# noirmist/Pytorch_Pose_Proposal_Network

Measured on AMD Instinct MI355X. Metric: images/sec (384x384, DRN-D-22) at 1/2/4/8 MI355X, higher is better.
Workload: dtype bf16

## Files before the change

pytorch_pose_proposal_network_amd/csrc/conv_big.hip:

```cpp
#include <algorithm>
#include <cstdio>
#include <cstdlib>
#include <type_traits>
#include <utility>

#include "conv_common.h"

namespace {

using namespace ppnconv;

constexpr bool stats_tile_ok(int bp, int bc) {
    return bc >= 128 && (size_t)bp * (size_t)(bc * 2 + 16) <= 2 * (size_t)(bp + bc) * 128;
}

#ifndef PPN_DIAG
#define PPN_DIAG 0
#endif
constexpr unsigned kOOB = 0x80000000u;

template <typename F, int... I>
__device__ __forceinline__ void static_for_impl(F&& f, std::integer_sequence<int, I...>) {
    (f(std::integral_constant<int, I>{}), ...);
}
template <int N, typename F>
__device__ __forceinline__ void static_for(F&& f) {
    static_for_impl(f, std::make_integer_sequence<int, N>{});
}

template <typename T>
__device__ __forceinline__ void load4(const char* p, float* v);
template <>
__device__ __forceinline__ void load4<float>(const char* p, float* v) {
    const float4 a = *reinterpret_cast<const float4*>(p);
    v[0] = a.x; v[1] = a.y; v[2] = a.z; v[3] = a.w;
}
template <>
__device__ __forceinline__ void load4<__bf16>(const char* p, float* v) {
    const uint2 a = *reinterpret_cast<const uint2*>(p);
    v[0] = __uint_as_float(a.x << 16); v[1] = __uint_as_float(a.x & 0xffff0000u);
    v[2] = __uint_as_float(a.y << 16); v[3] = __uint_as_float(a.y & 0xffff0000u);
}
template <>
__device__ __forceinline__ void load4<_Float16>(const char* p, float* v) {
    typedef __attribute__((ext_vector_type(4))) _Float16 f16x4;
    const f16x4 a = *reinterpret_cast<const f16x4*>(p);
#pragma unroll
    for (int i = 0; i < 4; ++i) v[i] = (float)a[i];
}
template <typename T>
__device__ __forceinline__ void store4(char* p, const float* v);
template <>
__device__ __forceinline__ void store4<float>(char* p, const float* v) {
    *reinterpret_cast<float4*>(p) = make_float4(v[0], v[1], v[2], v[3]);
}
template <>
__device__ __forceinline__ void store4<__bf16>(char* p, const float* v) {
    typedef __attribute__((ext_vector_type(4))) __bf16 bf16x4;
    bf16x4 o;
#pragma unroll
    for (int i = 0; i < 4; ++i) o[i] = (__bf16)v[i];
    *reinterpret_cast<bf16x4*>(p) = o;
}

template <>
__device__ __forceinline__ void store4<_Float16>(char* p, const float* v) {
    typedef __attribute__((ext_vector_type(4))) _Float16 f16x4;
    f16x4 o;
#pragma unroll
    for (int i = 0; i < 4; ++i) o[i] = (_Float16)clamp_f16(v[i]);
    *reinterpret_cast<f16x4*>(p) = o;
}

__device__ __forceinline__ void bufload_lds16(__amdgpu_buffer_rsrc_t rsrc, char* lds_wave_base, unsigned voff,
                                              unsigned soff) {
    __builtin_amdgcn_raw_ptr_buffer_load_lds(rsrc, (void __attribute__((address_space(3)))*)lds_wave_base, 16, voff,
                                             soff, 0, 0);
}

template <typename T, int BP, int BC, int NW, bool SC, bool X3 = false, bool ST = false, bool SP = false>
__global__ void __launch_bounds__(64 * NW, (ST && BP == 192 && BC == 128) ? 4 : NW / 4)
conv_igemm_big_kernel(ConvKArgs a, unsigned src_bytes, unsigned wgt_bytes) {
    static_assert(!X3 || (std::is_same<T, _Float16>::value && !SC), "X3 is the split-f16 mode without a fused shortcut");
    static_assert(!ST || (sizeof(T) == 2 && !SC && !X3 && NW == 8 && BC >= 128), "ST: plain 16-bit launches of the 8-wave tiles");
    static_assert(!SP || (sizeof(T) == 2 && BP == 192 && BC == 256 && NW == 8 && !SC && !X3 && !ST), "SP: the plain 16-bit 192 x 256 tile");
    constexpr int EPC = Elem<T>::EPC;
    constexpr int BK = 8 * EPC;
    constexpr int ES = sizeof(T);
    constexpr int NT = 64 * NW;
    constexpr int WC = (BP % (16 * (NW / 2)) == 0) ? 2 : NW;
    constexpr int WP = NW / WC;
    constexpr int NXI = (BP + 8 * NW - 1) / (8 * NW), NWI = BC / (8 * NW);
    constexpr bool XRAGGED = BP % (8 * NW) != 0;
    constexpr int TP = BP / WP / 16, TC = BC / WC / 16;
    constexpr int STAGE = (BP + BC) * 128;
    static_assert(BP % 8 == 0 && BC % (8 * NW) == 0 && (BP / WP) % 16 == 0 && BC % (16 * WC) == 0, "tile shape");
    static_assert(TP <= 9 && TC <= 8 && TC * TP % 2 == 0, "accumulators must fit the register file");

    extern __shared__ __attribute__((aligned(16))) char smem[];
#ifdef PPN_CLOCK
    const unsigned long long ck_entry = __builtin_amdgcn_s_memtime();
    const unsigned long long rk_entry = __builtin_amdgcn_s_memrealtime();
#endif
    const int tid = threadIdx.x, lane = tid & 63;
    const int wave = __builtin_amdgcn_readfirstlane(tid >> 6);
    const int wc = wave / WP, wp = wave % WP;

    int ptile, ctile;
    {
        const int nb = gridDim.x, id = blockIdx.x;
        const int xcd = id & 7, loc = id >> 3, q = nb >> 3, r = nb & 7;
        const int logical = (xcd < r ? xcd * (q + 1) : r * (q + 1) + (xcd - r) * q) + loc;
        ptile = fast_div(logical, a.div_nct);
        ctile = logical - ptile * a.n_ctiles;
    }
    const int m0 = a.m_base + ptile * BP, c0 = ctile * BC;

    const __amdgpu_buffer_rsrc_t xrs = __builtin_amdgcn_make_buffer_rsrc((void*)a.src, 0, src_bytes, 0x00020000);
    const __amdgpu_buffer_rsrc_t wrs = __builtin_amdgcn_make_buffer_rsrc((void*)a.wgt, 0, wgt_bytes, 0x00020000);
    const __amdgpu_buffer_rsrc_t xrs2 =
        __builtin_amdgcn_make_buffer_rsrc((void*)(SC ? a.src2 : a.src), 0, SC ? a.src2_bytes : 0u, 0x00020000);

    const int lrow = lane >> 3;
    const int chunk = (lane & 7) ^ (((lane >> 4) & 3) | ((wave & 1) << 2));
    const int ntaps = a.ks * a.ks;
    int xbase[NXI];
    int xbase2[NXI];
    unsigned xmask[NXI];
#pragma unroll
    for (int j = 0; j < NXI; ++j) {
        const int row = (j * NW + wave) * 8 + lrow;
        const int m = m0 + row;
        const bool vm = m < a.M;
        const int mm = vm ? m : 0;
        const int b = fast_div(mm, a.div_howo), rem = mm - b * a.HoWo;
        const int oy = fast_div(rem, a.div_wo), ox = rem - oy * a.Wo;
        const int iy0 = oy * a.stride - a.pad, ix0 = ox * a.stride - a.pad;
        xbase[j] = (((b * a.H + iy0) * a.W + ix0) * a.Cin + chunk * EPC) * ES;
        unsigned mk = 0, cx = 0;
#pragma unroll
        for (int dx = 0; dx < 5; ++dx)
            cx |= (dx < a.ks && (unsigned)(ix0 + dx * a.dil) < (unsigned)a.W) ? (1u << dx) : 0u;
#pragma unroll
        for (int dy = 0; dy < 5; ++dy)
            mk |= (dy < a.ks && (unsigned)(iy0 + dy * a.dil) < (unsigned)a.H) ? (cx << (dy * a.ks)) : 0u;
        mk = vm ? mk : 0u;
        xmask[j] = mk | (vm ? 0x80000000u : 0u);
        if constexpr (SC)
            xbase2[j] = (((b * a.H2 + oy * a.stride2) * a.W2 + ox * a.stride2) * a.Cin2 + chunk * EPC) * ES;
        else
            xbase2[j] = 0;
    }
    unsigned woff[NWI];
#pragma unroll
    for (int j = 0; j < NWI; ++j) {
        const int row = (j * NW + wave) * 8 + lrow;
        woff[j] = (unsigned)(((size_t)(c0 + row) * a.Ktot + chunk * EPC) * ES);
    }

    constexpr int SBUF = 256 * 128;
    constexpr int NSP = 4;
    int sbase[NSP];
    unsigned smask = 0;
    int xoff[TP][3];
    if constexpr (SP) {
        const int P = a.sp_pitch;
        const int schunk = (lane & 7) ^ (lrow & 6);
        const int b0 = fast_div(m0, a.div_howo), oy0 = fast_div(m0 - b0 * a.HoWo, a.div_wo);
#pragma unroll
        for (int p = 0; p < NSP; ++p) {
            const int sr = (p * NW + wave) * 8 + lrow;
            const int r = fast_div(sr, a.sp_div), col = sr - r * P;
            const int iy0 = oy0 + r - a.dil, ix = col - a.dil;
            sbase[p] = (((b0 * a.H + iy0) * a.W + ix) * a.Cin + schunk * EPC) * ES;
            const bool colok = r < a.sp_rows && (unsigned)ix < (unsigned)a.W;
#pragma unroll
            for (int dy = 0; dy < 3; ++dy)
                smask |= (colok && (unsigned)(iy0 + dy * a.dil) < (unsigned)a.H) ? (1u << (3 * p + dy)) : 0u;
        }
        const int fr = lane & 15, fqq = lane >> 4;
#pragma unroll
        for (int j = 0; j < TP; ++j) {
            const int ml = wp * (BP / WP) + j * 16 + fr;
            const int r = fast_div(ml, a.div_wo), rb = r * P + (ml - r * a.Wo);
#pragma unroll
            for (int dx = 0; dx < 3; ++dx) {
                const int row = rb + dx * a.dil;
                xoff[j][dx] = row * 128 + ((fqq ^ (row & 6)) << 4);
            }
        }
    }

    const int nsteps = a.Ktot / BK;
    const int dx_bytes = a.dil * a.Cin * ES;
    const int dy_bytes = a.dil * a.W * a.Cin * ES - a.ks * dx_bytes;
    const int ksz = a.ks;
    int u_tap = 0, u_dx = 0, u_slab = 0, tapoff = 0, u_ph = 0;
    unsigned tapbit = 1u;
    unsigned ksoff = 0;
    bool live = true;
    bool phase2 = a.nsteps_main == 0;
    int ld_step = 0;
    auto advance = [&]() {
        ++ld_step;
        live = ld_step < nsteps;
        ksoff = live ? ksoff + BK * ES : 0u;
        const bool now2 = SC && ld_step >= a.nsteps_main;
        if (!now2) {
            ++u_tap; ++u_dx;
            tapoff += dx_bytes;
            const bool wrapx = u_dx == ksz;
            u_dx = wrapx ? 0 : u_dx;
            tapoff += wrapx ? dy_bytes : 0;
            const bool wrapt = u_tap == ntaps;
            u_tap = wrapt ? 0 : u_tap;
            if constexpr (X3) {
                u_ph += wrapt ? 1 : 0;
                const bool wrapp = u_ph == 3;
                u_ph = wrapp ? 0 : u_ph;
                u_slab += wrapp ? BK * ES : 0;
                tapoff = wrapt ? u_slab + (u_ph == 2 ? a.lo_off : 0) : tapoff;
            } else {
                u_slab += wrapt ? BK * ES : 0;
                tapoff = wrapt ? u_slab : tapoff;
            }
            tapbit = live ? (1u << u_tap) : 0u;
        } else {
            tapoff = phase2 ? tapoff + BK * ES : 0;
            tapbit = live ? 0x80000000u : 0u;
        }
        phase2 = now2;
    };
    auto issue_one = [&](auto gc, int buf) {
        constexpr int g = decltype(gc)::value;
        char* xs = smem + buf * STAGE;
        if constexpr (g < NXI) {
            if constexpr (XRAGGED && g == NXI - 1)
                if ((g * NW + wave) * 8 >= BP) return;
            if (!SC || !phase2) {
                const unsigned voff = (xmask[g] & tapbit) ? (unsigned)(xbase[g] + tapoff) : kOOB;
                bufload_lds16(xrs, xs + (g * NW + wave) * 1024, voff, 0);
            } else {
                const unsigned voff = (xmask[g] & tapbit) ? (unsigned)(xbase2[g] + tapoff) : kOOB;
                bufload_lds16(xrs2, xs + (g * NW + wave) * 1024, voff, 0);
            }
        } else {
            constexpr int j = g - NXI;
            bufload_lds16(wrs, xs + BP * 128 + (j * NW + wave) * 1024, live ? woff[j] : kOOB, ksoff);
        }
    };
    constexpr int NL = NXI + NWI;
    const int sp_dy_bytes = a.dil * a.W * a.Cin * ES;
    const int sp_nq = nsteps / 3;
    int sp_row = 0, sp_dy = 0, sp_slab = 0, sp_off = 0;
    unsigned sp_bit = 1u;
    auto sp_advance_row = [&]() {
        ++sp_row; ++sp_dy;
        sp_off += sp_dy_bytes;
        const bool wrap = sp_dy == 3;
        sp_dy = wrap ? 0 : sp_dy;
        sp_slab += wrap ? BK * ES : 0;
        sp_off = wrap ? sp_slab : sp_off;
        sp_bit = sp_row < sp_nq ? (1u << sp_dy) : 0u;
    };
    auto sp_advance_w = [&]() {
        ++ld_step;
        live = ld_step < nsteps;
        ksoff = live ? ksoff + BK * ES : 0u;
    };
    auto sp_issue_strip = [&](auto pc, int sb) {
        constexpr int p = decltype(pc)::value;
        const unsigned voff = ((smask >> (3 * p)) & sp_bit) ? (unsigned)(sbase[p] + sp_off) : kOOB;
        bufload_lds16(xrs, smem + sb + (p * NW + wave) * 1024, voff, 0);
    };
    auto sp_issue_w = [&](auto jc, int buf) {
        constexpr int j = decltype(jc)::value;
        bufload_lds16(wrs, smem + 2 * SBUF + buf * (BC * 128) + (j * NW + wave) * 1024, live ? woff[j] : kOOB, ksoff);
    };

    const int frow = lane & 15, fq = lane >> 4;
    const int fswz = (frow >> 1) & 7;
    int foff[2];
    foff[0] = frow * 128 + (((0 + fq) ^ fswz) << 4);
    foff[1] = frow * 128 + (((4 + fq) ^ fswz) << 4);
    const int x_tile_off = wp * (BP / WP) * 128;
    const int w_tile_off = BP * 128 + wc * (BC / WC) * 128;

    f32x4 acc[TC][TP];
#pragma unroll
    for (int i = 0; i < TC; ++i)
#pragma unroll
        for (int j = 0; j < TP; ++j) acc[i][j] = f32x4{0.f, 0.f, 0.f, 0.f};

    f32x4 wA[TC], xA[TP], wB[TC], xB[TP];
    constexpr int NRD = TC + TP;
    auto read_one = [&](auto rc, f32x4 (&wf)[TC], f32x4 (&xf)[TP], int buf, int ks) {
        constexpr int r = decltype(rc)::value;
#if PPN_DIAG == 6
        if (buf >= 0 && ks >= 0 && nsteps > 0) { asm volatile("" : "+v"(xf[0]), "+v"(wf[0])); return; }
#endif
        if constexpr (r < TP)
            xf[r] = *reinterpret_cast<const f32x4*>(smem + buf * STAGE + x_tile_off + foff[ks] + r * 16 * 128);
        else
            wf[r - TP] = *reinterpret_cast<const f32x4*>(smem + buf * STAGE + w_tile_off + foff[ks] + (r - TP) * 16 * 128);
    };
    auto sp_read_one = [&](auto rc, auto dxc, f32x4 (&wf)[TC], f32x4 (&xf)[TP], int wbuf, int xsel, int ks) {
        constexpr int r = decltype(rc)::value;
        constexpr int DX = decltype(dxc)::value;
        if constexpr (r < TP)
            xf[r] = *reinterpret_cast<const f32x4*>(smem + (xoff[r][DX] ^ xsel));
        else
            wf[r - TP] = *reinterpret_cast<const f32x4*>(smem + 2 * SBUF + wbuf * (BC * 128) + wc * (BC / WC) * 128 + foff[ks] +
                                                         (r - TP) * 16 * 128);
    };
    constexpr int GS = (TC * TP % 4 == 0) ? 4 : ((TC * TP % 3 == 0) ? 3 : 2);
    constexpr int NG = TC * TP / GS;
#if PPN_DIAG == 3 || PPN_DIAG == 4
    typedef float f32x16 __attribute__((ext_vector_type(16)));
    f32x16 acc32[TC * TP / 4];
#pragma unroll
    for (int i = 0; i < TC * TP / 4; ++i)
#pragma unroll
        for (int j = 0; j < 16; ++j) acc32[i][j] = 0.f;
#endif
    auto mma_group = [&](auto gc, const f32x4 (&wf)[TC], const f32x4 (&xf)[TP]) {
        constexpr int g = decltype(gc)::value;
#if PPN_DIAG == 3 || PPN_DIAG == 4
        if constexpr (std::is_same<T, __bf16>::value) {
            constexpr int i0 = g * 4, i1 = g * 4 + 3;
            acc32[g] = __builtin_amdgcn_mfma_f32_32x32x16_bf16(__builtin_bit_cast(bf16x8, wf[i0 / TP]),
                                                               __builtin_bit_cast(bf16x8, xf[i0 % TP]), acc32[g], 0, 0, 0);
            acc32[g] = __builtin_amdgcn_mfma_f32_32x32x16_bf16(__builtin_bit_cast(bf16x8, wf[i1 / TP]),
                                                               __builtin_bit_cast(bf16x8, xf[i1 % TP]), acc32[g], 0, 0, 0);
            return;
        }
#endif
        static_for<GS>([&](auto tc) {
            constexpr int idx = g * GS + decltype(tc)::value;
            mma_step(acc[idx / TP][idx % TP], wf[idx / TP], xf[idx % TP], (T*)nullptr);
        });
    };
    constexpr int RPG = (NRD + NG - 1) / NG;
    constexpr int LPG = (NL + NG - 1) / NG;

#ifdef PPN_CLOCK
    const unsigned long long ck_state = __builtin_amdgcn_s_memtime();
#endif
    if constexpr (SP) {
        static_for<NSP>([&](auto pc) { sp_issue_strip(pc, 0); });
        static_for<NWI>([&](auto jc) { sp_issue_w(jc, 0); });
        sp_advance_row();
        sp_advance_w();
        static_for<2>([&](auto pc) { sp_issue_strip(pc, SBUF); });
        static_for<NWI>([&](auto jc) { sp_issue_w(jc, 1); });
        sp_advance_w();
        asm volatile("s_waitcnt vmcnt(%0)" ::"n"(NWI + 2) : "memory");
    } else {
        static_for<NL>([&](auto gc) { issue_one(gc, 0); });
        advance();
        static_for<NL>([&](auto gc) { issue_one(gc, 1); });
        advance();
        if constexpr (XRAGGED) {
            if ((NXI - 1) * NW * 8 + wave * 8 < BP) asm volatile("s_waitcnt vmcnt(%0)" ::"n"(NL) : "memory");
            else asm volatile("s_waitcnt vmcnt(%0)" ::"n"(NL - 1) : "memory");
        } else {
            asm volatile("s_waitcnt vmcnt(%0)" ::"n"(NL) : "memory");
        }
    }
    __syncthreads();
#ifdef PPN_CLOCK
    const unsigned long long ck_bar = __builtin_amdgcn_s_memtime();
#endif
    if constexpr (SP) {
        constexpr std::integral_constant<int, 0> dx0{};
        static_for<NRD>([&](auto rc) { sp_read_one(rc, dx0, wA, xA, 0, 0, 0); });
        static_for<NRD>([&](auto rc) { sp_read_one(rc, dx0, wB, xB, 0, 64, 1); });
    } else {
        static_for<NRD>([&](auto rc) { read_one(rc, wA, xA, 0, 0); });
        static_for<NRD>([&](auto rc) { read_one(rc, wB, xB, 0, 1); });
    }
    static_for<NG>([&](auto gc) { mma_group(gc, wA, xA); });
    asm volatile("s_waitcnt vmcnt(0) lgkmcnt(0)" ::: "memory");
    __syncthreads();

#ifdef PPN_STAMP
    unsigned long long st_b1 = 0, st_b2 = 0, st_wait = 0, st_bar = 0, tq0, tq1;
#define PPN_T(var) do { __builtin_amdgcn_sched_barrier(0); asm volatile("s_memtime %0\n\ts_waitcnt lgkmcnt(0)" : "=s"(var) :: "memory"); __builtin_amdgcn_sched_barrier(0); } while (0)
#else
#define PPN_T(var) do { } while (0)
#endif
#ifdef PPN_CLOCK
    const unsigned long long ck0 = __builtin_amdgcn_s_memtime(), rk0 = __builtin_amdgcn_s_memrealtime();
#endif
    if constexpr (SP) {
        int s = 1, sbo = 0;
        auto step = [&](auto dxc) {
            constexpr int DX = decltype(dxc)::value;
            constexpr int NS = DX == 0 ? 2 : 1;
            const int buf = s & 1;
            static_for<NG>([&](auto gc) {
                constexpr int g = decltype(gc)::value;
                mma_group(gc, wB, xB);
                if constexpr (g < NS) sp_issue_strip(std::integral_constant<int, (DX == 0 ? g : DX + 1)>{}, sbo ^ SBUF);
                else if constexpr (g < NS + NWI) sp_issue_w(std::integral_constant<int, g - NS>{}, buf ^ 1);
                static_for<RPG>([&](auto rc) {
                    constexpr int r = g * RPG + decltype(rc)::value;
                    if constexpr (r < NRD) sp_read_one(std::integral_constant<int, r>{}, dxc, wA, xA, buf, sbo, 0);
                });
                __builtin_amdgcn_sched_barrier(0);
            });
            sp_advance_w();
            static_for<NG>([&](auto gc) {
                constexpr int g = decltype(gc)::value;
                mma_group(gc, wA, xA);
                static_for<RPG>([&](auto rc) {
                    constexpr int r = g * RPG + decltype(rc)::value;
                    if constexpr (r < NRD) sp_read_one(std::integral_constant<int, r>{}, dxc, wB, xB, buf, sbo | 64, 1);
                });
                __builtin_amdgcn_sched_barrier(0);
            });
            asm volatile("s_waitcnt vmcnt(0) lgkmcnt(0)" ::: "memory");
            __syncthreads();
            ++s;
        };
        static_assert(NG >= 2 + NWI, "one DMA per MFMA group");
        for (int q = 1; q < sp_nq; ++q) {
            step(std::integral_constant<int, 1>{});
            step(std::integral_constant<int, 2>{});
            sbo ^= SBUF;
            sp_advance_row();
            step(std::integral_constant<int, 0>{});
        }
        step(std::integral_constant<int, 1>{});
        step(std::integral_constant<int, 2>{});
    } else
    for (int s = 1; s < nsteps; ++s) {
        const int buf = s & 1;
#ifdef PPN_STAMP
        PPN_T(tq0);
#endif
        static_for<NG>([&](auto gc) {
            constexpr int g = decltype(gc)::value;
            mma_group(gc, wB, xB);
#if PPN_DIAG != 2 && PPN_DIAG != 4 && PPN_DIAG != 5 && PPN_DIAG != 6
            static_for<LPG>([&](auto lc) {
                constexpr int l = g * LPG + decltype(lc)::value;
                if constexpr (l < NL) issue_one(std::integral_constant<int, l>{}, buf ^ 1);
            });
#endif
            static_for<RPG>([&](auto rc) {
                constexpr int r = g * RPG + decltype(rc)::value;
                if constexpr (r < NRD) read_one(std::integral_constant<int, r>{}, wA, xA, buf, 0);
            });
            __builtin_amdgcn_sched_barrier(0);
        });
        advance();
#ifdef PPN_STAMP
        PPN_T(tq1); st_b1 += tq1 - tq0;
#endif
        static_for<NG>([&](auto gc) {
            constexpr int g = decltype(gc)::value;
            mma_group(gc, wA, xA);
            static_for<RPG>([&](auto rc) {
                constexpr int r = g * RPG + decltype(rc)::value;
                if constexpr (r < NRD) read_one(std::integral_constant<int, r>{}, wB, xB, buf, 1);
            });
            __builtin_amdgcn_sched_barrier(0);
        });
#ifdef PPN_STAMP
        PPN_T(tq0); st_b2 += tq0 - tq1;
#endif
#if PPN_DIAG == 1
        asm volatile("s_waitcnt lgkmcnt(0)" ::: "memory");
#else
        asm volatile("s_waitcnt vmcnt(0) lgkmcnt(0)" ::: "memory");
#endif
#ifdef PPN_STAMP
        PPN_T(tq1); st_wait += tq1 - tq0;
#endif
#if PPN_DIAG != 5
        __syncthreads();
#endif
#ifdef PPN_STAMP
        PPN_T(tq0); st_bar += tq0 - tq1;
#endif
    }
#ifdef PPN_CLOCK
    {
        const unsigned long long ck1 = __builtin_amdgcn_s_memtime(), rk1 = __builtin_amdgcn_s_memrealtime();
        if (lane == 0 && a.scale2 == nullptr && a.shift2 != nullptr) {
            unsigned long long* dbg = (unsigned long long*)a.shift2 + ((size_t)blockIdx.x * NW + wave) * 8;
            dbg[0] = ck1 - ck0; dbg[1] = rk1 - rk0; dbg[2] = ck0 - ck_entry; dbg[3] = ck1; dbg[5] = ck_state - ck_entry; dbg[6] = ck_bar - ck_entry;
        }
    }
#endif
#ifdef PPN_STAMP
    unsigned long long t_epi0;
    PPN_T(t_epi0);
    if (lane == 0 && a.scale2 == nullptr && a.shift2 != nullptr) {
        unsigned long long* dbg = (unsigned long long*)a.shift2 + ((size_t)blockIdx.x * NW + wave) * 8;
        dbg[0] = st_b1; dbg[1] = st_b2; dbg[2] = st_wait; dbg[3] = st_bar;
    }
#endif
    static_for<NG>([&](auto gc) { mma_group(gc, wB, xB); });
#if PPN_DIAG == 3 || PPN_DIAG == 4
#pragma unroll
    for (int i = 0; i < TC * TP / 4; ++i)
#pragma unroll
        for (int j = 0; j < 16; ++j) acc[(i * 4 + j / 4) / TP][(i * 4 + j / 4) % TP][j % 4] += acc32[i][j];
#endif
    __syncthreads();

    int pf_keep0 = 0, pf_keep1 = 0;
    if (a.pf_per_wg) {
        const unsigned l0 = blockIdx.x * a.pf_per_wg + tid, lend = min((blockIdx.x + 1) * a.pf_per_wg, a.pf_lines);
        if (l0 < lend) pf_keep0 = *reinterpret_cast<const int*>(a.pf_ptr + (size_t)l0 * 128);
        if (l0 + 64 * NW < lend) pf_keep1 = *reinterpret_cast<const int*>(a.pf_ptr + (size_t)(l0 + 64 * NW) * 128);
        asm volatile("" : "+v"(pf_keep0), "+v"(pf_keep1));
    }

    float* ct = reinterpret_cast<float*>(smem);
    constexpr int RS16 = BC * 2 + 16;
#ifdef PPN_NO_FAST_EPI
    constexpr bool kFastFits = false;
#else
    constexpr bool kFastFits = !X3 && sizeof(T) == 2 && BC >= 128 && (size_t)BP * RS16 <= 2 * (size_t)STAGE;
#endif
#ifndef PPN_NO_FAST_EPI
    static_assert(!ST || kFastFits, "ST lives in the single-output 16-bit epilogue");
#endif
    bool fast = false;
    if constexpr (kFastFits) fast = !a.nchw && !a.residual && !a.out_act && a.out_raw && (a.Cout & 7) == 0 && !a.out_bf16;
    if (fast) {
        if constexpr (kFastFits) {
            const float slope1 = a.act1 == PPN_ACT_RELU ? 0.f : (a.act1 == PPN_ACT_LRELU ? 0.1f : 1.f);
            const bool al = (!a.scale1 || (reinterpret_cast<size_t>(a.scale1) & 15) == 0) &&
                            (!a.shift1 || (reinterpret_cast<size_t>(a.shift1) & 15) == 0);
#pragma unroll
            for (int i = 0; i < TC; ++i) {
                const int chl = wc * (BC / WC) + i * 16 + 4 * fq;
                const int c = c0 + chl;
                float sc[4] = {1.f, 1.f, 1.f, 1.f}, sh[4] = {0.f, 0.f, 0.f, 0.f};
                if (al && c + 4 <= a.Cout) {
                    if (a.scale1) { const float4 t = *reinterpret_cast<const float4*>(a.scale1 + c); sc[0] = t.x; sc[1] = t.y; sc[2] = t.z; sc[3] = t.w; }
                    if (a.shift1) { const float4 t = *reinterpret_cast<const float4*>(a.shift1 + c); sh[0] = t.x; sh[1] = t.y; sh[2] = t.z; sh[3] = t.w; }
                } else {
#pragma unroll
                    for (int r = 0; r < 4; ++r) {
                        if (a.scale1 && c + r < a.Cout) sc[r] = a.scale1[c + r];
                        if (a.shift1 && c + r < a.Cout) sh[r] = a.shift1[c + r];
                    }
                }
#pragma unroll
                for (int j = 0; j < TP; ++j) {
                    const int px = wp * (BP / WP) + j * 16 + frow;
                    float v[4];
#pragma unroll
                    for (int r = 0; r < 4; ++r) {
                        const float t1 = acc[i][j][r] * sc[r] + sh[r];
                        v[r] = fmaxf(t1, t1 * slope1);
                    }
                    store4<T>(smem + px * RS16 + chl * 2, v);
                }
            }
            constexpr int CPR = BC / 8;
            constexpr int NQ = BP * CPR / NT;
            static_assert(BP * CPR % NT == 0, "tile must split into whole 16-byte chunks per thread");
            const size_t row_bytes = (size_t)a.Cout * 2;
            static_assert(!ST || NT % CPR == 0, "ST: a thread keeps its chunk column");
            uint4 sx[ST ? NQ : 1];
            float st_sc[8], st_sh[8], st_mu[8], st_rs[8], st_s0[8], st_s1[8];
            float st_neg = 1.f;
            const int st_mode = ST ? a.st_mode : 0;
            if constexpr (ST) {
#pragma unroll
                for (int j = 0; j < 8; ++j) st_s0[j] = st_s1[j] = 0.f;
                if (st_mode == 2) {
                    const int cc = tid % CPR, c = c0 + cc * 8;
                    const bool vc = c < a.Cout;
                    static_for<NQ>([&](auto qc) {
                        constexpr int q = decltype(qc)::value;
                        const int m = m0 + q * (NT / CPR) + tid / CPR;
                        sx[q] = (vc && m < a.M) ? *reinterpret_cast<const uint4*>(a.st_x + (size_t)m * row_bytes + (size_t)c * 2)
                                                : make_uint4(0u, 0u, 0u, 0u);
                    });
                    const int cb = vc ? c : 0;
                    float ga[8], be[8];
                    auto vec8 = [&](const float* p, float* o) {
                        if ((reinterpret_cast<size_t>(p) & 15) == 0) {
                            const float4 lo = *reinterpret_cast<const float4*>(p + cb), hi = *reinterpret_cast<const float4*>(p + cb + 4);
                            o[0] = lo.x; o[1] = lo.y; o[2] = lo.z; o[3] = lo.w; o[4] = hi.x; o[5] = hi.y; o[6] = hi.z; o[7] = hi.w;
                        } else {
#pragma unroll
                            for (int j = 0; j < 8; ++j) o[j] = p[cb + j];
                        }
                    };
                    vec8(a.st_mean, st_mu); vec8(a.st_rstd, st_rs); vec8(a.st_gamma, ga); vec8(a.st_beta, be);
#pragma unroll
                    for (int j = 0; j < 8; ++j) {
                        st_sc[j] = ga[j] * st_rs[j];
                        st_sh[j] = be[j] - st_mu[j] * st_sc[j];
                    }
                    st_neg = a.st_act == PPN_ACT_RELU ? 0.f : (a.st_act == PPN_ACT_LRELU ? 0.1f : 1.f);
                }
            }
            lds_barrier();
            auto store_chunk = [&](auto qc, auto modec) {
                constexpr int q = decltype(qc)::value;
                constexpr int MODE = decltype(modec)::value;
                const int id = q * NT + tid;
                const int px = id / CPR, cc = id % CPR;
                const int m = m0 + px, c = c0 + cc * 8;
                if (m < a.M && c < a.Cout) {
                    const uint4 o = *reinterpret_cast<const uint4*>(smem + px * RS16 + cc * 16);
                    *reinterpret_cast<uint4*>(a.out_raw + (size_t)m * row_bytes + (size_t)c * 2) = o;
                    if constexpr (MODE != 0) {
                        float v[8];
                        load8<T>(reinterpret_cast<const char*>(&o), v);
                        if constexpr (MODE == 1) {
#pragma unroll
                            for (int j = 0; j < 8; ++j) {
                                st_s0[j] += v[j];
                                st_s1[j] = fmaf(v[j], v[j], st_s1[j]);
                            }
                        } else {
                            float x[8];
                            load8<T>(reinterpret_cast<const char*>(&sx[q]), x);
#pragma unroll
                            for (int j = 0; j < 8; ++j) {
                                const float z = fmaf(x[j], st_sc[j], st_sh[j]);
                                const float g = v[j] * (z > 0.f ? 1.f : st_neg);
                                const float xh = (x[j] - st_mu[j]) * st_rs[j];
                                st_s0[j] += g;
                                st_s1[j] = fmaf(g, xh, st_s1[j]);
                            }
                        }
                    }
                }
            };
            if constexpr (!ST) {
#pragma unroll
                for (int q = 0; q < NQ; ++q) {
                    const int id = q * NT + tid;
                    const int px = id / CPR, cc = id % CPR;
                    const int m = m0 + px, c = c0 + cc * 8;
                    if (m < a.M && c < a.Cout) {
                        const uint4 o = *reinterpret_cast<const uint4*>(smem + px * RS16 + cc * 16);
                        *reinterpret_cast<uint4*>(a.out_raw + (size_t)m * row_bytes + (size_t)c * 2) = o;
                    }
                }
            } else {
                if (st_mode == 0) static_for<NQ>([&](auto qc) { store_chunk(qc, std::integral_constant<int, 0>{}); });
                if (st_mode == 1) static_for<NQ>([&](auto qc) { store_chunk(qc, std::integral_constant<int, 1>{}); });
                if (st_mode == 2) static_for<NQ>([&](auto qc) { store_chunk(qc, std::integral_constant<int, 2>{}); });
            }
            if constexpr (ST) {
                if (st_mode != 0) {
#pragma unroll
                    for (int off = 32; off >= CPR; off >>= 1)
#pragma unroll
                        for (int j = 0; j < 8; ++j) {
                            st_s0[j] += __shfl_xor(st_s0[j], off, 64);
                            st_s1[j] += __shfl_xor(st_s1[j], off, 64);
                        }
                    lds_barrier();
                    float* red = reinterpret_cast<float*>(smem);
                    if (lane < CPR) {
#pragma unroll
                        for (int j = 0; j < 8; ++j) {
                            red[(wave * CPR + lane) * 16 + j] = st_s0[j];
                            red[(wave * CPR + lane) * 16 + 8 + j] = st_s1[j];
                        }
                    }
                    lds_barrier();
                    if (tid < CPR * 16) {
                        const int ccx = tid >> 4, j = tid & 15;
                        double acc = 0.0;
#pragma unroll
                        for (int w = 0; w < NW; ++w) acc += (double)red[(w * CPR + ccx) * 16 + j];
                        const int ch = c0 + ccx * 8 + (j & 7);
                        if (ch < a.Cout) a.st_partial[((size_t)ptile * a.Cout + ch) * 2 + (j >> 3)] = acc;
                    }
                }
            }
        }
// ... 122 lines not shown
            const unsigned long long e2 = __builtin_amdgcn_s_memtime();
            ep_w += e1 - e0; ep_s += e2 - e1;
#endif
        };
        static_for<TP / JC>(chunk);
#ifdef PPN_CLOCK
        if (lane == 0 && a.scale2 == nullptr && a.shift2 != nullptr) {
            unsigned long long* dbg = (unsigned long long*)a.shift2 + ((size_t)blockIdx.x * NW + wave) * 8;
            dbg[7] = (ep_w << 32) | ep_s;
        }
#endif
    } else {
        constexpr int LD = BP + 4;
        constexpr int IC = WC == 2 ? 2 : 1;
        constexpr int TPC = BP / 4;
        constexpr int NITEM = WC * IC * 16 * TPC;
        static_assert(TC % IC == 0, "channel tiles per wave must be even");
        static_assert((size_t)(WC * IC * 16 * LD + 4 * IC * 16) * 4 <= 2 * (size_t)STAGE, "epilogue chunk must fit the staging LDS");
        float* out = reinterpret_cast<float*>(a.out_raw);
        const bool vec = (a.HoWo & 3) == 0;
        auto chunk = [&](auto qc) {
            constexpr int q = decltype(qc)::value;
#pragma unroll
            for (int ii = 0; ii < IC; ++ii) {
                const int chl = (wc * IC + ii) * 16 + 4 * fq;
                const int c = c0 + wc * (BC / WC) + (q * IC + ii) * 16 + 4 * fq;
                float sc[4], sh[4];
#pragma unroll
                for (int r = 0; r < 4; ++r) {
                    sc[r] = (a.scale1 && c + r < a.Cout) ? a.scale1[c + r] : 1.f;
                    sh[r] = (a.shift1 && c + r < a.Cout) ? a.shift1[c + r] : 0.f;
                }
#pragma unroll
                for (int j = 0; j < TP; ++j) {
                    const int px = wp * (BP / WP) + j * 16 + frow;
#pragma unroll
                    for (int r = 0; r < 4; ++r) ct[(chl + r) * LD + px] = acc[q * IC + ii][j][r] * sc[r] + sh[r];
                }
            }
            lds_barrier();
#if PPN_DIAG == 8
            if (a.amax_keys && a.M < 0) {
#else
            if (a.amax_keys) {
#endif
                constexpr int RUN = IC * 16;
                const int nedges = (a.Cout - a.unary_ch) / a.window;
                for (int item = tid; item < WC * BP; item += NT) {
                    const int cw = item / BP, px = item - cw * BP;
                    const int m = m0 + px;
                    if (m >= a.M) continue;
                    const int nb = fast_div(m, a.div_howo), np = m - nb * a.HoWo;
                    const int cb = c0 + cw * (BC / WC) + q * RUN;
                    const float* row = ct + (cw * RUN) * LD + px;
                    int r = 0;
                    for (; r < RUN && cb + r < a.unary_ch; ++r)
                        a.unary_out[((size_t)nb * a.unary_ch + cb + r) * a.HoWo + np] = sigmoid_fast(row[r * LD]);
                    const int rend = min(RUN, a.Cout - cb);
                    if (r < rend) {
                        const int l0 = cb + r - a.unary_ch;
                        int e = l0 / a.window, sidx = l0 - e * a.window;
                        while (r < rend) {
                            const int seg = min(rend - r, a.window - sidx);
                            float tm = -3.0e38f, tm2 = -3.0e38f;
                            int km = 0;
#pragma unroll 8
                            for (int k = 0; k < seg; ++k) {
                                const float t = row[(r + k) * LD];
                                tm2 = fmaxf(tm2, fminf(tm, t));
                                const bool gt = t > tm;
                                tm = gt ? t : tm;
                                km = gt ? k : km;
                            }
                            float best = sigmoid_fast(tm);
                            int best_k = km;
                            if (!(tm2 < tm - 9.5367431640625e-7f * (1.0f + __expf(tm)))) {
                                best = -1.f;
                                best_k = 0;
                                for (int k = 0; k < seg; ++k) {
                                    const float v = sigmoid_fast(row[(r + k) * LD]);
                                    const bool gt = v > best;
                                    best = gt ? v : best;
                                    best_k = gt ? k : best_k;
                                }
                            }
#if PPN_DIAG == 9
                            if (e < nedges && best == 12345.678f) {
#else
                            if (e < nedges) {
#endif
                                const unsigned long long key = ((unsigned long long)__float_as_uint(best) << 32) |
                                                               (unsigned)(0xFFFFFFFFu - (unsigned)(sidx + best_k));
                                atomicMax(a.amax_keys + ((size_t)nb * nedges + e) * a.HoWo + np, key);
                            }
                            r += seg; sidx = 0; ++e;
                        }
                    }
                }
            }
            if (out)
            for (int item = tid; item < NITEM; item += NT) {
                const int chl = item / TPC, pq = item - chl * TPC;
                const int cw = chl / (IC * 16), ci = (chl / 16) % IC, cr = chl % 16;
                const int c = c0 + cw * (BC / WC) + (q * IC + ci) * 16 + cr;
                const int m = m0 + 4 * pq;
                if (c < a.Cout && m < a.M) {
                    const f32x4 t4 = *reinterpret_cast<const f32x4*>(ct + chl * LD + 4 * pq);
                    float v[4] = {t4.x, t4.y, t4.z, t4.w};
#pragma unroll
                    for (int i = 0; i < 4; ++i) v[i] = apply_act(v[i], a.act1);
                    if (vec) {
                        const int nb = fast_div(m, a.div_howo), np = m - nb * a.HoWo;
                        *reinterpret_cast<float4*>(out + ((size_t)nb * a.Cout + c) * a.HoWo + np) =
                            make_float4(v[0], v[1], v[2], v[3]);
                    } else {
#pragma unroll
                        for (int i = 0; i < 4; ++i) {
                            const int mi = m + i;
                            if (mi < a.M) {
                                const int bi = fast_div(mi, a.div_howo), pi = mi - bi * a.HoWo;
                                out[((size_t)bi * a.Cout + c) * a.HoWo + pi] = v[i];
                            }
                        }
                    }
                }
            }
            lds_barrier();
        };
        static_for<TC / IC>(chunk);
    }
    asm volatile("" ::"v"(pf_keep0), "v"(pf_keep1));
#ifdef PPN_CLOCK
    if (lane == 0 && a.scale2 == nullptr && a.shift2 != nullptr) {
        unsigned long long* dbg = (unsigned long long*)a.shift2 + ((size_t)blockIdx.x * NW + wave) * 8;
        dbg[4] = __builtin_amdgcn_s_memtime() - dbg[3];
#if PPN_CLOCK + 0 >= 2
        dbg[5] = rk_entry; dbg[6] = __builtin_amdgcn_s_memrealtime();
#endif
    }
    (void)rk_entry;
#endif
#ifdef PPN_STAMP
    {
        unsigned long long t_epi1;
        PPN_T(t_epi1);
        if (lane == 0 && a.scale2 == nullptr && a.shift2 != nullptr) {
            unsigned long long* dbg = (unsigned long long*)a.shift2 + ((size_t)blockIdx.x * NW + wave) * 8;
            dbg[4] = t_epi1 - t_epi0;
        }
    }
#endif
}

template <typename T, int BP, int BC, int NW, bool SC, bool X3 = false, bool ST = false, bool SP = false>
int launch_sc(const ConvKArgs& a, hipStream_t st, const char** kname) {
    constexpr size_t lds = SP ? 2 * (size_t)(256 + BC) * 128 : 2 * (size_t)(BP + BC) * 128;
    static char name[96];
    if (!name[0])
        snprintf(name, sizeof(name), "conv_igemm_big_kernel<%s, %d, %d, %d, %s%s>", elem_name<T>(),
                 BP, BC, NW, SC ? "true" : "false", X3 ? ", true" : (ST ? ", false, true" : ""));
    if (kname) *kname = name;
    const size_t src_bytes = (size_t)a.B * a.H * a.W * a.Cin * sizeof(T);
    const size_t wgt_bytes = (size_t)a.n_ctiles * BC * a.Ktot * sizeof(T);
    auto k = conv_igemm_big_kernel<T, BP, BC, NW, SC, X3, ST, SP>;
    {
        static int max_lds_set = 0;
        PPN_LDS_ONCE(max_lds_set, reinterpret_cast<const void*>(k), hipFuncAttributeMaxDynamicSharedMemorySize,
                                      (int)lds);
    }
    ConvKArgs b = a;
    if (b.pf_lines) {
        const unsigned nwg = (unsigned)(a.n_ctiles * a.n_ptiles);
        b.pf_per_wg = std::min<unsigned>((b.pf_lines + nwg - 1) / nwg, 2u * 64 * NW);
    }
    hipLaunchKernelGGL(k, dim3(a.n_ctiles * a.n_ptiles), dim3(64 * NW), lds, st, b, (unsigned)src_bytes,
                       (unsigned)wgt_bytes);
    PPN_LAUNCH_CHECK();
    return PPN_OK;
}

template <typename T, int BP, int BC, int NW>
int launch_one(const ConvKArgs& a, hipStream_t st, const char** kname) {
    if constexpr (NW == 8 && BC >= 128) {
        if (a.src2) return launch_sc<T, BP, BC, NW, true>(a, st, kname);
    } else {
        if (a.src2) return ppn::fail(PPN_E_UNSUPPORTED, "fused shortcut needs the 8-wave 128/256-channel tiles");
    }
    if (a.st_mode != 0) {
        if constexpr (std::is_same<T, __bf16>::value && NW == 8 && stats_tile_ok(BP, BC))
            return launch_sc<T, BP, BC, NW, false, false, true>(a, st, kname);
        else
            return ppn::fail(PPN_E_UNSUPPORTED, "BatchNorm statistics: no such instantiation of the large-tile kernel");
    }
    if constexpr (sizeof(T) == 2 && BP == 192 && BC == 256 && NW == 8) {
        if (a.sp_rows > 0) return launch_sc<T, BP, BC, NW, false, false, false, true>(a, st, kname);
    }
    return launch_sc<T, BP, BC, NW, false>(a, st, kname);
}

int conv_waves() {
    static const int nw = getenv("PPN_CONV_WAVES") ? atoi(getenv("PPN_CONV_WAVES")) : 8;
    return nw;
}

template <typename T>
int launch_T(const ConvKArgs& a, BigTile t, hipStream_t st, const char** kname) {
    const int nw = conv_waves();
    if (nw == 4 && t.bp != 144) {
        if (t.bc == 256) {
            if (t.bp == 256) return launch_one<T, 256, 256, 4>(a, st, kname);
            if (t.bp == 192) return launch_one<T, 192, 256, 4>(a, st, kname);
            return launch_one<T, 128, 256, 4>(a, st, kname);
        }
        if (t.bp == 256) return launch_one<T, 256, 128, 4>(a, st, kname);
        if (t.bp == 192) return launch_one<T, 192, 128, 4>(a, st, kname);
        return launch_one<T, 128, 128, 4>(a, st, kname);
    }
    if (t.bc == 256) {
        if (t.bp == 256) return launch_one<T, 256, 256, 8>(a, st, kname);
        if (t.bp == 192) return launch_one<T, 192, 256, 8>(a, st, kname);
        if (t.bp == 144) return launch_one<T, 144, 256, 8>(a, st, kname);
        return launch_one<T, 128, 256, 8>(a, st, kname);
    }
    if (t.bc == 128) {
        if (t.bp == 256) return launch_one<T, 256, 128, 8>(a, st, kname);
        if (t.bp == 192) return launch_one<T, 192, 128, 8>(a, st, kname);
        return launch_one<T, 128, 128, 8>(a, st, kname);
    }
    if (t.bp == 256) return launch_one<T, 256, 64, 8>(a, st, kname);
    return launch_one<T, 128, 64, 8>(a, st, kname);
}

int launch_X3(const ConvKArgs& a, BigTile t, hipStream_t st, const char** kname) {
    if (a.src2) return ppn::fail(PPN_E_UNSUPPORTED, "PPN_F16X3: no fused shortcut");
    if (t.bc == 256) {
        if (t.bp == 256) return launch_sc<_Float16, 256, 256, 8, false, true>(a, st, kname);
        if (t.bp == 192) return launch_sc<_Float16, 192, 256, 8, false, true>(a, st, kname);
        if (t.bp == 144) return launch_sc<_Float16, 144, 256, 8, false, true>(a, st, kname);
        return launch_sc<_Float16, 128, 256, 8, false, true>(a, st, kname);
    }
    if (t.bc == 128) {
        if (t.bp == 256) return launch_sc<_Float16, 256, 128, 8, false, true>(a, st, kname);
        if (t.bp == 192) return launch_sc<_Float16, 192, 128, 8, false, true>(a, st, kname);
        return launch_sc<_Float16, 128, 128, 8, false, true>(a, st, kname);
    }
    if (t.bp == 256) return launch_sc<_Float16, 256, 64, 8, false, true>(a, st, kname);
    return launch_sc<_Float16, 128, 64, 8, false, true>(a, st, kname);
}

}

namespace ppnconv {

static int g_tile_policy = getenv("PPN_CONV_CONT") ? 1 : 0;
static int g_ov_bp = -1, g_ov_bc = 0;

static bool tile_shape_ok(int bp, int bc) {
    if (bp == 144) return bc == 256;
    return (bp == 128 || bp == 192 || bp == 256) && (bc == 64 || bc == 128 || bc == 256) && !(bc == 64 && bp == 192);
}

static const double kEff144 = getenv("PPN_EFF144") ? atof(getenv("PPN_EFF144")) : 0.90;

bool big_tile_for(int cout, long long m, BigTile* out, int ksteps, bool shared_gpu) {
    if (cout < 64) return false;
    if (g_ov_bp < 0) {
        g_ov_bp = g_ov_bc = 0;
        int bp = 0, bc = 0;
        const char* ov = getenv("PPN_CONV_TILE");
        if (ov && sscanf(ov, "%d,%d", &bp, &bc) == 2 && tile_shape_ok(bp, bc)) { g_ov_bp = bp; g_ov_bc = bc; }
    }
    if (g_ov_bp > 0 && g_ov_bc <= ((cout + 63) / 64) * 64 && g_ov_bc <= (cout >= 256 ? 256 : (cout >= 128 ? 128 : 64))) {
        out->bp = g_ov_bp; out->bc = g_ov_bc;
        return true;
    }
    if (cout >= 4096) {
        out->bp = 192; out->bc = 128;
        return true;
    }
    struct Cand { int bp, bc; double eff; };
    static const Cand cands[] = {{256, 256, 1.27}, {192, 256, 1.10}, {144, 256, kEff144}, {128, 256, 0.92}, {256, 128, 0.90},
                                 {192, 128, 0.95}, {128, 128, 0.87}, {256, 64, 0.60},  {128, 64, 0.55}};
    int bc_max = cout >= 256 ? 256 : (cout >= 128 ? 128 : 64);
    const int bc_min = cout >= 256 ? 128 : bc_max;
    if (ksteps > 0 && ksteps <= 8 && bc_max == 256) bc_max = 128;
    double best = 1e30;
    for (const Cand& cd : cands) {
        if (cd.bc > bc_max || cd.bc < bc_min || cd.eff <= 0.0 || (shared_gpu && cd.bp == 144)) continue;
        const long long tiles = ((m + cd.bp - 1) / cd.bp) * ((cout + cd.bc - 1) / cd.bc);
        static const int p1mask = getenv("PPN_POLICY1_MASK") ? atoi(getenv("PPN_POLICY1_MASK")) : 7;
        const int cls = cout >= 512 ? (m >= 65536 ? 1 : 2) : 4;
        const bool frac = g_tile_policy == 1 && (p1mask & cls);
        const double rounds = frac ? (double)tiles / 256.0 : (double)((tiles + 255) / 256);
        const double cost = rounds * cd.bp * cd.bc / cd.eff;
        if (cost < best) { best = cost; out->bp = cd.bp; out->bc = cd.bc; }
    }
    return true;
}

long long big_split_for(int cout, long long m) {
    BigTile single;
    if (g_tile_policy != 2 || cout < 256 || cout >= 4096 || !big_tile_for(cout, m, &single) || g_ov_bp > 0) return 0;
    struct Cand { int bp, bc; double eff; };
    static const Cand cands[] = {{256, 256, 1.27}, {192, 256, 1.10}, {128, 256, 0.92}, {256, 128, 0.90},
                                 {192, 128, 0.95}, {128, 128, 0.87}};
    auto rounds_cost = [&](const Cand& cd, long long mm) {
        const long long tiles = ((mm + cd.bp - 1) / cd.bp) * ((cout + cd.bc - 1) / cd.bc);
        return (double)((tiles + 255) / 256) * cd.bp * cd.bc / cd.eff;
    };
    double best_single = 1e30;
    for (const Cand& cd : cands) best_single = std::min(best_single, rounds_cost(cd, m));
    double best = best_single * 0.96;
    long long cut = 0;
    for (const Cand& p : cands) {
        const long long ct = (cout + p.bc - 1) / p.bc;
        if (256 % ct != 0) continue;
        const long long rounds = (m / p.bp) * ct / 256;
        if (rounds < 1) continue;
        const long long m1 = rounds * 256 / ct * p.bp;
        if (m1 >= m) continue;
        double tail = 1e30;
        for (const Cand& q : cands) tail = std::min(tail, rounds_cost(q, m - m1));
        const double cost = (double)rounds * p.bp * p.bc / p.eff + tail;
        if (cost < best) { best = cost; cut = m1; }
    }
    return cut;
}

bool big_stats_ok(int dtype, BigTile t) {
    return dtype == PPN_BF16 && conv_waves() == 8 && stats_tile_ok(t.bp, t.bc);
}

static int g_strip_on = -1;
thread_local int g_last_strip = 0;

static bool strip_eligible(const ConvKArgs& a, int dtype, BigTile t, int* rows, int* pitch) {
    if (g_strip_on < 0) g_strip_on = (getenv("PPN_CONV_STRIP") && atoi(getenv("PPN_CONV_STRIP")) == 0) ? 0 : 1;
    if (!g_strip_on || conv_waves() != 8 || t.bp != 192 || t.bc != 256 || (dtype != PPN_BF16 && dtype != PPN_F16)) return false;
    if (a.ks != 3 || a.stride != 1 || a.dil < 1 || a.pad != a.dil || a.Ho != a.H || a.Wo != a.W || a.Ktot != 9 * a.Cin) return false;
    if (a.src2 || a.st_mode != 0 || a.nchw || a.amax_keys || a.unary_out) return false;
    if (192 % a.Wo != 0 || a.HoWo % 192 != 0 || a.m_base % 192 != 0 || (a.M - a.m_base) % 192 != 0) return false;
    const int r = 192 / a.Wo, p = a.Wo + 8 * ((2 * a.dil + 7) / 8);
    if (r * p > 256) return false;
    *rows = r; *pitch = p;
    return true;
}

// ... 36 lines not shown
```

Measured before the change: 11830.

## Add residual epilogue for strip conv with LDS-staged residual prefetch and coalesced stores

Adds an RS variant of the 192x256 strip kernel, used when a residual add is present and Cout is a multiple of 256. During the last main-loop step it DMAs residual tiles into LDS and loads the per-channel affine tables. The epilogue then applies BN, activation and the residual add, plus an optional second affine and activation, in LDS and writes 16-byte coalesced rows. The goal is to hide residual-load latency behind the final MFMAs and avoid scattered global stores. The cost is a larger LDS footprint (5x32KB) and hand-tuned vmcnt counts that could be fragile.

```diff
diff --git a/pytorch_pose_proposal_network_amd/csrc/conv_big.hip b/pytorch_pose_proposal_network_amd/csrc/conv_big.hip
--- a/pytorch_pose_proposal_network_amd/csrc/conv_big.hip
+++ b/pytorch_pose_proposal_network_amd/csrc/conv_big.hip
@@ -78,11 +78,40 @@
                                              soff, 0, 0);
 }
 
-template <typename T, int BP, int BC, int NW, bool SC, bool X3 = false, bool ST = false, bool SP = false>
+typedef __attribute__((ext_vector_type(2))) unsigned u32x2;
+typedef __attribute__((ext_vector_type(4))) unsigned u32x4;
+__device__ __forceinline__ unsigned lds_addr(const char* p) {
+    return (unsigned)(size_t)(const __attribute__((address_space(3))) char*)p;
+}
+__device__ __forceinline__ void rs_read_tile(unsigned ra, unsigned ta, u32x2& res, ppnconv::f32x4& sc, ppnconv::f32x4& sh) {
+    asm volatile("ds_read_b64 %0, %3\n\tds_read_b128 %1, %4\n\tds_read_b128 %2, %4 offset:2048\n\ts_waitcnt lgkmcnt(0)"
+                 : "=&v"(res), "=&v"(sc), "=&v"(sh) : "v"(ra), "v"(ta) : "memory");
+}
+__device__ __forceinline__ void rs_read_affine(unsigned ta, ppnconv::f32x4& sc, ppnconv::f32x4& sh) {
+    asm volatile("ds_read_b128 %0, %2\n\tds_read_b128 %1, %2 offset:2048\n\ts_waitcnt lgkmcnt(0)"
+                 : "=&v"(sc), "=&v"(sh) : "v"(ta) : "memory");
+}
+__device__ __forceinline__ void rs_write8(unsigned addr, u32x2 v) {
+    asm volatile("ds_write_b64 %0, %1" ::"v"(addr), "v"(v) : "memory");
+}
+__device__ __forceinline__ void rs_read_rows(unsigned addr, u32x4& o0, u32x4& o1, u32x4& o2, u32x4& o3) {
+    asm volatile("ds_read_b128 %0, %4\n\tds_read_b128 %1, %4 offset:8192\n\tds_read_b128 %2, %4 offset:16384\n\t"
+                 "ds_read_b128 %3, %4 offset:24576\n\ts_waitcnt lgkmcnt(0)"
+                 : "=&v"(o0), "=&v"(o1), "=&v"(o2), "=&v"(o3) : "v"(addr) : "memory");
+}
+template <typename T>
+__device__ __forceinline__ u32x2 pack4(const float* v) {
+    u32x2 o;
+    store4<T>(reinterpret_cast<char*>(&o), v);
+    return o;
+}
+
+template <typename T, int BP, int BC, int NW, bool SC, bool X3 = false, bool ST = false, bool SP = false, bool RS = false>
 __global__ void __launch_bounds__(64 * NW, (ST && BP == 192 && BC == 128) ? 4 : NW / 4)
 conv_igemm_big_kernel(ConvKArgs a, unsigned src_bytes, unsigned wgt_bytes) {
     static_assert(!X3 || (std::is_same<T, _Float16>::value && !SC), "X3 is the split-f16 mode without a fused shortcut");
     static_assert(!ST || (sizeof(T) == 2 && !SC && !X3 && NW == 8 && BC >= 128), "ST: plain 16-bit launches of the 8-wave tiles");
+    static_assert(!RS || SP, "RS: the residual epilogue of the strip launches");
     static_assert(!SP || (sizeof(T) == 2 && BP == 192 && BC == 256 && NW == 8 && !SC && !X3 && !ST), "SP: the plain 16-bit 192 x 256 tile");
     constexpr int EPC = Elem<T>::EPC;
     constexpr int BK = 8 * EPC;
@@ -191,6 +220,7 @@
         }
     }
 
+    float rs_t0 = 1.f, rs_t1 = 0.f;
     const int nsteps = a.Ktot / BK;
     const int dx_bytes = a.dil * a.Cin * ES;
     const int dy_bytes = a.dil * a.W * a.Cin * ES - a.ks * dx_bytes;
@@ -278,6 +308,15 @@
         bufload_lds16(wrs, smem + 2 * SBUF + buf * (BC * 128) + (j * NW + wave) * 1024, live ? woff[j] : kOOB, ksoff);
     };
 
+    const __amdgpu_buffer_rsrc_t rrs = __builtin_amdgcn_make_buffer_rsrc(
+        (void*)(RS ? a.residual : a.src), 0, RS ? (unsigned)a.B * (unsigned)a.HoWo * (unsigned)a.Cout * 2u : 0u, 0x00020000);
+    auto rs_issue = [&](int q, int p, int dst) {
+        const int rrow = wave * 2 + (lane >> 5);
+        const int rc = c0 + (((lane & 31) ^ rrow) << 3);
+        const unsigned voff = rc < a.Cout ? (unsigned)(((m0 + rrow) * a.Cout + rc) * 2) : kOOB;
+        bufload_lds16(rrs, smem + dst + (p * NW + wave) * 1024, voff, (unsigned)((p * 48 + q * 16) * a.Cout * 2));
+    };
+
     const int frow = lane & 15, fq = lane >> 4;
     const int fswz = (frow >> 1) & 7;
     int foff[2];
@@ -394,13 +433,17 @@
 #endif
     if constexpr (SP) {
         int s = 1, sbo = 0;
-        auto step = [&](auto dxc) {
+        auto step = [&](auto dxc, auto lastc) {
             constexpr int DX = decltype(dxc)::value;
+            constexpr bool LAST = RS && decltype(lastc)::value;
             constexpr int NS = DX == 0 ? 2 : 1;
             const int buf = s & 1;
             static_for<NG>([&](auto gc) {
                 constexpr int g = decltype(gc)::value;
                 mma_group(gc, wB, xB);
+                if constexpr (LAST) {
+                    if constexpr (g < 4) rs_issue(0, g, 4 * SBUF);
+                } else
                 if constexpr (g < NS) sp_issue_strip(std::integral_constant<int, (DX == 0 ? g : DX + 1)>{}, sbo ^ SBUF);
                 else if constexpr (g < NS + NWI) sp_issue_w(std::integral_constant<int, g - NS>{}, buf ^ 1);
                 static_for<RPG>([&](auto rc) {
@@ -424,15 +467,24 @@
             ++s;
         };
         static_assert(NG >= 2 + NWI, "one DMA per MFMA group");
+        constexpr std::false_type inner{};
         for (int q = 1; q < sp_nq; ++q) {
-            step(std::integral_constant<int, 1>{});
-            step(std::integral_constant<int, 2>{});
+            step(std::integral_constant<int, 1>{}, inner);
+            step(std::integral_constant<int, 2>{}, inner);
             sbo ^= SBUF;
             sp_advance_row();
-            step(std::integral_constant<int, 0>{});
-        }
-        step(std::integral_constant<int, 1>{});
-        step(std::integral_constant<int, 2>{});
+            step(std::integral_constant<int, 0>{}, inner);
+        }
+        step(std::integral_constant<int, 1>{}, inner);
+        if constexpr (RS) {
+            const int tch = c0 + (tid & 255);
+            const bool second = wave >= NW / 2;
+            const float* ps = !second ? a.scale1 : (a.out_act ? a.scale2 : nullptr);
+            const float* pb = !second ? a.shift1 : (a.out_act ? a.shift2 : nullptr);
+            rs_t0 = (ps && tch < a.Cout) ? ps[tch] : 1.f;
+            rs_t1 = (pb && tch < a.Cout) ? pb[tch] : 0.f;
+        }
+        step(std::integral_constant<int, 2>{}, std::true_type{});
     } else
     for (int s = 1; s < nsteps; ++s) {
         const int buf = s & 1;
@@ -502,6 +554,13 @@
         dbg[0] = st_b1; dbg[1] = st_b2; dbg[2] = st_wait; dbg[3] = st_bar;
     }
 #endif
+    if constexpr (RS) {
+        float* tab = reinterpret_cast<float*>(smem + 3 * SBUF);
+        tab[tid] = rs_t0;
+        tab[512 + tid] = rs_t1;
+        static_for<4>([&](auto pc) { rs_issue(1, decltype(pc)::value, 0); });
+        static_for<4>([&](auto pc) { rs_issue(2, decltype(pc)::value, SBUF); });
+    }
     static_for<NG>([&](auto gc) { mma_group(gc, wB, xB); });
 #if PPN_DIAG == 3 || PPN_DIAG == 4
 #pragma unroll
@@ -509,9 +568,23 @@
 #pragma unroll
         for (int j = 0; j < 16; ++j) acc[(i * 4 + j / 4) / TP][(i * 4 + j / 4) % TP][j % 4] += acc32[i][j];
 #endif
+    if constexpr (RS) lds_barrier();
+    else
     __syncthreads();
 
     int pf_keep0 = 0, pf_keep1 = 0;
+    if constexpr (RS) {
+        if (a.pf_per_wg) {
+            const unsigned l0 = blockIdx.x * a.pf_per_wg + tid, lend = min((blockIdx.x + 1) * a.pf_per_wg, a.pf_lines);
+            const __amdgpu_buffer_rsrc_t prs = __builtin_amdgcn_make_buffer_rsrc(
+                (void*)a.pf_ptr, 0, (unsigned)min((unsigned long long)a.pf_lines * 128ull, 0x7fffff00ull), 0x00020000);
+            char* pl = smem + 3 * SBUF + 4096 + wave * 256;
+            __builtin_amdgcn_raw_ptr_buffer_load_lds(prs, (void __attribute__((address_space(3)))*)pl, 4,
+                                                     l0 < lend ? l0 * 128u : kOOB, 0, 0, 0);
+            __builtin_amdgcn_raw_ptr_buffer_load_lds(prs, (void __attribute__((address_space(3)))*)(pl + 2048), 4,
+                                                     l0 + 64 * NW < lend ? (l0 + 64 * NW) * 128u : kOOB, 0, 0, 0);
+        }
+    } else
     if (a.pf_per_wg) {
         const unsigned l0 = blockIdx.x * a.pf_per_wg + tid, lend = min((blockIdx.x + 1) * a.pf_per_wg, a.pf_lines);
         if (l0 < lend) pf_keep0 = *reinterpret_cast<const int*>(a.pf_ptr + (size_t)l0 * 128);
@@ -531,6 +604,87 @@
 #endif
     bool fast = false;
     if constexpr (kFastFits) fast = !a.nchw && !a.residual && !a.out_act && a.out_raw && (a.Cout & 7) == 0 && !a.out_bf16;
+    if constexpr (RS) {
+        const float slope1 = a.act1 == PPN_ACT_RELU ? 0.f : (a.act1 == PPN_ACT_LRELU ? 0.1f : 1.f);
+        const float slope2 = a.act2 == PPN_ACT_RELU ? 0.f : (a.act2 == PPN_ACT_LRELU ? 0.1f : 1.f);
+        const bool two = a.out_act != nullptr;
+        const unsigned lds0 = lds_addr(smem);
+        const unsigned tab = lds0 + 3 * SBUF;
+        const int eoff = (wp * 16 + frow) * 512 + (fq & 1) * 8;
+        const unsigned soff = (unsigned)((tid >> 5) * 512 + (((tid & 31) ^ (tid >> 5)) << 4));
+        const size_t row_bytes = (size_t)a.Cout * 2;
+        const size_t goff0 = (size_t)(m0 + (tid >> 5)) * row_bytes + (size_t)(c0 + (tid & 31) * 8) * 2;
+#ifdef PPN_CLOCK
+        unsigned long long ep_w = 0, ep_s = 0;
+#endif
+        static_for<3>([&](auto qc) {
+            constexpr int q = decltype(qc)::value;
+            constexpr int RB = q == 0 ? 4 * SBUF : (q - 1) * SBUF;
+#ifdef PPN_CLOCK
+            const unsigned long long e0 = __builtin_amdgcn_s_memtime();
+#endif
+            if constexpr (q > 0) {
+                if (two) asm volatile("s_waitcnt vmcnt(%0) lgkmcnt(0)\n\ts_barrier" ::"n"(q == 1 ? 12 : 16) : "memory");
+                else asm volatile("s_waitcnt vmcnt(%0) lgkmcnt(0)\n\ts_barrier" ::"n"(8) : "memory");
+            }
+#ifdef PPN_CLOCK
+            const unsigned long long e1 = __builtin_amdgcn_s_memtime();
+#endif
+#pragma unroll
+            for (int i = 0; i < TC; ++i) {
+                const int chl = wc * (BC / WC) + i * 16 + 4 * fq;
+                const int pos = eoff + (((chl >> 3) ^ frow) << 4);
+                u32x2 rbits;
+                f32x4 sc, sh;
+                rs_read_tile(lds0 + RB + pos, tab + chl * 4, rbits, sc, sh);
+                float res[4], v[4];
+                load4<T>(reinterpret_cast<const char*>(&rbits), res);
+#pragma unroll
+                for (int r = 0; r < 4; ++r) {
+                    const float t1 = acc[i][q][r] * sc[r] + sh[r];
+                    v[r] = fmaxf(t1, t1 * slope1) + res[r];
+                }
+                rs_write8(lds0 + RB + pos, pack4<T>(v));
+                if (two) {
+                    f32x4 sc2, sh2;
+                    rs_read_affine(tab + 1024 + chl * 4, sc2, sh2);
+                    float u[4];
+#pragma unroll
+                    for (int r = 0; r < 4; ++r) {
+                        const float t2 = v[r] * sc2[r] + sh2[r];
+                        u[r] = fmaxf(t2, t2 * slope2);
+                    }
+                    rs_write8(lds0 + 2 * SBUF + pos, pack4<T>(u));
+                }
+            }
+            lds_barrier();
+#ifdef PPN_CLOCK
+            const unsigned long long e2 = __builtin_amdgcn_s_memtime();
+#endif
+            {
+                u32x4 o[4];
+                rs_read_rows(lds0 + RB + soff, o[0], o[1], o[2], o[3]);
+#pragma unroll
+                for (int pass = 0; pass < 4; ++pass)
+                    *reinterpret_cast<u32x4*>(a.out_raw + goff0 + (size_t)(pass * (BP / WP) + q * 16) * row_bytes) = o[pass];
+                if (two) {
+                    rs_read_rows(lds0 + 2 * SBUF + soff, o[0], o[1], o[2], o[3]);
+#pragma unroll
+                    for (int pass = 0; pass < 4; ++pass)
+                        *reinterpret_cast<u32x4*>(a.out_act + goff0 + (size_t)(pass * (BP / WP) + q * 16) * row_bytes) = o[pass];
+                }
+            }
+#ifdef PPN_CLOCK
+            ep_w += e1 - e0; ep_s += __builtin_amdgcn_s_memtime() - e2;
+#endif
+        });
+#ifdef PPN_CLOCK
+        if (lane == 0 && a.scale2 == nullptr && a.shift2 != nullptr) {
+            unsigned long long* dbg = (unsigned long long*)a.shift2 + ((size_t)blockIdx.x * NW + wave) * 8;
+            dbg[7] = (1ull << 63) | (ep_w << 32) | ep_s;
+        }
+#endif
+    } else
     if (fast) {
         if constexpr (kFastFits) {
             const float slope1 = a.act1 == PPN_ACT_RELU ? 0.f : (a.act1 == PPN_ACT_LRELU ? 0.1f : 1.f);
@@ -959,9 +1113,10 @@
 #endif
 }
 
-template <typename T, int BP, int BC, int NW, bool SC, bool X3 = false, bool ST = false, bool SP = false>
+template <typename T, int BP, int BC, int NW, bool SC, bool X3 = false, bool ST = false, bool SP = false, bool RS = false>
 int launch_sc(const ConvKArgs& a, hipStream_t st, const char** kname) {
-    constexpr size_t lds = SP ? 2 * (size_t)(256 + BC) * 128 : 2 * (size_t)(BP + BC) * 128;
+    constexpr size_t lds = RS ? 5 * (size_t)256 * 128 : SP ? 2 * (size_t)(256 + BC) * 128 : 2 * (size_t)(BP + BC) * 128;
+    static_assert(!RS || 2 * (256 + BC) * 128 == 4 * 256 * 128, "RS: the epilogue's LDS map");
     static char name[96];
     if (!name[0])
         snprintf(name, sizeof(name), "conv_igemm_big_kernel<%s, %d, %d, %d, %s%s>", elem_name<T>(),
@@ -969,7 +1124,7 @@
     if (kname) *kname = name;
     const size_t src_bytes = (size_t)a.B * a.H * a.W * a.Cin * sizeof(T);
     const size_t wgt_bytes = (size_t)a.n_ctiles * BC * a.Ktot * sizeof(T);
-    auto k = conv_igemm_big_kernel<T, BP, BC, NW, SC, X3, ST, SP>;
+    auto k = conv_igemm_big_kernel<T, BP, BC, NW, SC, X3, ST, SP, RS>;
     {
         static int max_lds_set = 0;
         PPN_LDS_ONCE(max_lds_set, reinterpret_cast<const void*>(k), hipFuncAttributeMaxDynamicSharedMemorySize,
@@ -984,6 +1139,12 @@
                        (unsigned)wgt_bytes);
     PPN_LAUNCH_CHECK();
     return PPN_OK;
+}
+
+bool rs_eligible(const ConvKArgs& a) {
+    if (!a.residual || !a.out_raw || a.out_bf16 || a.Cout % 256 != 0) return false;
+    if ((size_t)a.B * a.HoWo * a.Cout * 2 >= 0x7fffff00ull) return false;
+    return ((reinterpret_cast<size_t>(a.residual) | reinterpret_cast<size_t>(a.out_raw) | reinterpret_cast<size_t>(a.out_act)) & 15) == 0;
 }
 
 template <typename T, int BP, int BC, int NW>
@@ -1000,6 +1161,7 @@
             return ppn::fail(PPN_E_UNSUPPORTED, "BatchNorm statistics: no such instantiation of the large-tile kernel");
     }
     if constexpr (sizeof(T) == 2 && BP == 192 && BC == 256 && NW == 8) {
+        if (a.sp_rows > 0 && rs_eligible(a)) return launch_sc<T, BP, BC, NW, false, false, false, true, true>(a, st, kname);
         if (a.sp_rows > 0) return launch_sc<T, BP, BC, NW, false, false, false, true>(a, st, kname);
     }
     return launch_sc<T, BP, BC, NW, false>(a, st, kname);
```

New measurement: 11970 (median of 6 runs). Within noise of the previous version (+1.2%).
